# mratsim/constantine

Measured on NVIDIA H100. Metric: bls12_381_g1_msm_throughput, higher is better.
Workload: dtype u32

## Files before the change

### constantine_b200/_lib.py

```python
import ctypes
import os

_HERE = os.path.dirname(os.path.abspath(__file__))
LIB_PATH = os.environ.get("CTT_B200_LIB", os.path.join(_HERE, "lib", "libctt_b200_msm.so"))
_lib = None


class Stats(ctypes.Structure):
    _fields_ = [("c", ctypes.c_int), ("num_windows", ctypes.c_int),
                ("entries", ctypes.c_ulonglong), ("total_buckets", ctypes.c_ulonglong),
                ("kernel_launches", ctypes.c_int),
                ("ms_h2d", ctypes.c_float), ("ms_digits", ctypes.c_float), ("ms_sort", ctypes.c_float),
                ("ms_accumulate", ctypes.c_float), ("ms_fixup", ctypes.c_float), ("ms_reduce", ctypes.c_float),
                ("ms_d2h_tail", ctypes.c_float), ("ms_total", ctypes.c_float),
                ("groups", ctypes.c_int), ("slice_len", ctypes.c_int), ("affine_levels", ctypes.c_int),
                ("ms_affine", ctypes.c_float)]


def load():
    global _lib
    if _lib is not None:
        return _lib
    if not os.path.exists(LIB_PATH):
        raise RuntimeError(
# ... 27 lines not shown
    lib.ctt_b200_msm_batch_cached_bases.restype = ci
    lib.ctt_b200_bases_precompute_for.argtypes = [vp, sz, ci]
    lib.ctt_b200_bases_precompute_for.restype = ci
    lib.ctt_b200_sum_reduce_host.argtypes = [ci, ci, vp, vp, sz]
    lib.ctt_b200_sum_reduce_host.restype = ci
    lib.ctt_b200_last_stats.argtypes = [ctypes.POINTER(Stats)]
    lib.ctt_b200_last_stats.restype = None
    lib.ctt_b200_set_tuning.argtypes = [ci, ci, ci]
    lib.ctt_b200_set_tuning.restype = None
    lib.ctt_b200_set_concurrency.argtypes = [ci]
    lib.ctt_b200_set_concurrency.restype = None
    lib.ctt_b200_set_groups.argtypes = [ci]
    lib.ctt_b200_set_groups.restype = None
    lib.ctt_b200_set_affine_levels.argtypes = [ci]
    lib.ctt_b200_set_affine_levels.restype = None
    lib.ctt_b200_set_reduce_mode.argtypes = [ci]
    lib.ctt_b200_set_reduce_mode.restype = None
    lib.ctt_b200_set_input_chunks.argtypes = [ci]
    lib.ctt_b200_set_input_chunks.restype = None
    lib.ctt_b200_set_point_chunks.argtypes = [ci]
    lib.ctt_b200_set_point_chunks.restype = None
    lib.ctt_b200_set_stream.argtypes = [vp]
    lib.ctt_b200_set_stream.restype = None
    lib.ctt_b200_sm_count.argtypes = []
    lib.ctt_b200_sm_count.restype = ci
    lib.ctt_b200_set_devices.argtypes = [ctypes.POINTER(ci), ci]
    lib.ctt_b200_set_devices.restype = ci
    lib.ctt_b200_device_count.argtypes = []
    lib.ctt_b200_device_count.restype = ci
    lib.ctt_b200_test_field_op.argtypes = [ci, ci, vp, vp, vp, sz]
# ... 58 lines not shown
```

### constantine_b200/csrc/msm_affine.cuh

```cuda
#pragma once
#include "ec.cuh"
#include "field_inv.cuh"

namespace b200 {

constexpr int AFF_MAX_LEVELS = 8;
constexpr uint32_t AFF_NONE = 0xFFFFFFFFu;

static __global__ void k_bucket_bounds(const uint32_t* __restrict__ keys, size_t n, uint32_t no_key, uint32_t* head, uint32_t* tail) {
  size_t q = (size_t)blockIdx.x * blockDim.x + threadIdx.x;
  if (q >= n) return;
  const uint32_t key = keys[q];
  if (key >= no_key) return;
  if (q == 0 || keys[q - 1] != key) head[key] = (uint32_t)q;
  if (q + 1 == n || keys[q + 1] != key) tail[key] = (uint32_t)(q + 1);
}

constexpr int SCAN_THREADS = 256, SCAN_PER_THREAD = 4, SCAN_ITEMS = SCAN_THREADS * SCAN_PER_THREAD;

B200_DEV uint32_t block_exclusive_scan(uint32_t v, uint32_t& total, uint32_t* smem ) {
  const unsigned lane = threadIdx.x & 31u, warp = threadIdx.x >> 5;
  uint32_t inc = v;
#pragma unroll
  for (int d = 1; d < 32; d <<= 1) {
    uint32_t t = __shfl_up_sync(0xFFFFFFFFu, inc, d);
    if (lane >= (unsigned)d) inc += t;
  }
  __syncthreads();
  if (lane == 31u) smem[warp] = inc;
  __syncthreads();
  uint32_t base = 0, tot = 0;
#pragma unroll
  for (int w = 0; w < SCAN_THREADS / 32; w++) {
    const uint32_t s = smem[w];
    if ((unsigned)w < warp) base += s;
    tot += s;
  }
  total = tot;
  return base + inc - v;
}

B200_DEV uint32_t level_count(uint32_t n, int r) { return (n + (1u << r) - 1u) >> r; }

static __global__ void __launch_bounds__(SCAN_THREADS) k_level_blocksums(const uint32_t* __restrict__ head, const uint32_t* __restrict__ tail,
                                                                          uint32_t nb, int L, uint32_t nblk, uint32_t* blocksum ) {
  __shared__ uint32_t sm[SCAN_THREADS / 32 + 1];
  const uint32_t b0 = blockIdx.x * SCAN_ITEMS + threadIdx.x * SCAN_PER_THREAD;
  uint32_t cnt[SCAN_PER_THREAD];
#pragma unroll
  for (int k = 0; k < SCAN_PER_THREAD; k++) cnt[k] = (b0 + k < nb) ? tail[b0 + k] - head[b0 + k] : 0u;
  for (int r = 0; r <= L; r++) {
    uint32_t s = 0;
#pragma unroll
    for (int k = 0; k < SCAN_PER_THREAD; k++) s += level_count(cnt[k], r);
    uint32_t tot;
    block_exclusive_scan(s, tot, sm);
    if (threadIdx.x == 0) blocksum[(size_t)r * nblk + blockIdx.x] = tot;
  }
}

static __global__ void __launch_bounds__(SCAN_THREADS) k_level_scan(uint32_t* blocksum, uint32_t nblk, int L, uint32_t nb, uint32_t* off) {
  __shared__ uint32_t sm[SCAN_THREADS / 32 + 1];
  for (int r = 0; r <= L; r++) {
    uint32_t carry = 0;
    for (uint32_t base = 0; base < nblk; base += SCAN_THREADS) {
// ... 3 lines not shown
      const uint32_t ex = block_exclusive_scan(v, tot, sm);
      if (i < nblk) blocksum[(size_t)r * nblk + i] = carry + ex;
      carry += tot;
    }
    if (threadIdx.x == 0) off[(size_t)r * (nb + 1) + nb] = carry;
  }
}

static __global__ void __launch_bounds__(SCAN_THREADS) k_level_offsets(const uint32_t* __restrict__ head, const uint32_t* __restrict__ tail,
                                                                        uint32_t nb, int L, uint32_t nblk, const uint32_t* __restrict__ blocksum,
                                                                        uint32_t* off) {
  __shared__ uint32_t sm[SCAN_THREADS / 32 + 1];
  const uint32_t b0 = blockIdx.x * SCAN_ITEMS + threadIdx.x * SCAN_PER_THREAD;
  uint32_t cnt[SCAN_PER_THREAD];
#pragma unroll
  for (int k = 0; k < SCAN_PER_THREAD; k++) cnt[k] = (b0 + k < nb) ? tail[b0 + k] - head[b0 + k] : 0u;
  for (int r = 0; r <= L; r++) {
    uint32_t c[SCAN_PER_THREAD], s = 0;
#pragma unroll
    for (int k = 0; k < SCAN_PER_THREAD; k++) { c[k] = level_count(cnt[k], r); s += c[k]; }
    uint32_t tot;
    uint32_t ex = block_exclusive_scan(s, tot, sm) + blocksum[(size_t)r * nblk + blockIdx.x];
#pragma unroll
    for (int k = 0; k < SCAN_PER_THREAD; k++) {
      if (b0 + k < nb) off[(size_t)r * (nb + 1) + b0 + k] = ex;
      ex += c[k];
    }
  }
}

struct AffinePlan {
  uint2* plan0;
  uint32_t* plan[AFF_MAX_LEVELS];
  uint32_t* surv_keys;
  uint32_t* surv_vals;
};

static __global__ void k_affine_plan(const uint32_t* __restrict__ keys, const uint32_t* __restrict__ vals, size_t n, uint32_t no_key,
                                     const uint32_t* __restrict__ head, const uint32_t* __restrict__ tail,
                                     const uint32_t* __restrict__ off, uint32_t nb, int L, AffinePlan P) {
  size_t q = (size_t)blockIdx.x * blockDim.x + threadIdx.x;
  if (q >= n) return;
  const uint32_t b = keys[q];
  if (b >= no_key) return;
  const uint32_t h = head[b], i = (uint32_t)q - h, cnt = tail[b] - h;
  const size_t stride = (size_t)nb + 1;
  for (int r = 0; r < L; r++) {
    if (i & ((2u << r) - 1u)) break;
    const uint32_t p = off[(size_t)(r + 1) * stride + b] + (i >> (r + 1));
    const uint32_t s = i >> r;
    const bool has2 = s + 1u < level_count(cnt, r);
    if (r == 0) P.plan0[p] = make_uint2(vals[q], has2 ? vals[q + 1] : AFF_NONE);
    else P.plan[r][p] = (off[(size_t)r * stride + b] + s) | (has2 ? 0x80000000u : 0u);
  }
  if ((i & ((1u << L) - 1u)) == 0u) {
    const uint32_t ps = off[(size_t)L * stride + b] + (i >> L);
    P.surv_keys[ps] = b;
    P.surv_vals[ps] = ps;
  }
}

template <class T>
B200_DEV Aff<T> load_affine_rw(const uint32_t* base, size_t idx) {
  const uint32_t* p = base + idx * (2 * T::WORDS);
  Aff<T> a;
  load_words_rw(a.x, p);
  load_words_rw(a.y, p + T::WORDS);
  return a;
}
template <class T>
B200_DEV void store_affine(uint32_t* base, size_t idx, const Aff<T>& a) {
  uint32_t* p = base + idx * (2 * T::WORDS);
  store_words(p, a.x);
  store_words(p + T::WORDS, a.y);
// ... 291 lines not shown
```

### constantine_b200/csrc/msm_capi.cu

```cuda
#define CTT_B200_BUILDING_LIBRARY
#include "../../include/ctt_b200_msm.h"
#include "msm_hooks.cuh"
#include <thread>

namespace b200 {
B200_DECLARE_CURVE(Bls12381G1) B200_DECLARE_CURVE(Bn254G1) B200_DECLARE_CURVE(PallasEc) B200_DECLARE_CURVE(VestaEc)
B200_DECLARE_CURVE(Bls12381G2) B200_DECLARE_CURVE(Bn254G2)
B200_DECLARE_FIELD(Bls12381Fp) B200_DECLARE_FIELD(Bn254SnarksFp) B200_DECLARE_FIELD(PallasFp) B200_DECLARE_FIELD(VestaFp)
B200_DECLARE_FIELD(Bls12381Fr) B200_DECLARE_FIELD(Bn254SnarksFr) B200_DECLARE_FIELD(PallasFr) B200_DECLARE_FIELD(VestaFr)

struct Bases {
  int curve_id;
  size_t len;
  void* d_points;
  void* d_table = nullptr;
  int table_c = 0, table_W = 0;
};

void bases_view(const ctt_b200_bases* bases, const void** d_points, size_t* table_stride, int* force_c) {
  const Bases* b = reinterpret_cast<const Bases*>(bases);
  *d_points = b->d_table ? b->d_table : b->d_points;
  *table_stride = b->d_table ? b->len : 0;
  *force_c = b->d_table ? b->table_c : 0;
}
// ... 209 lines not shown
  if (slice_len < -1) cfg.tuning.slice_len = slice_len;
}

void ctt_b200_set_groups(int groups) {
  Config& cfg = config();
  std::lock_guard<std::mutex> lock(cfg.mu);
  cfg.tuning.groups = groups < 0 ? 0 : groups;
}

void ctt_b200_set_affine_levels(int levels) {
  Config& cfg = config();
  std::lock_guard<std::mutex> lock(cfg.mu);
  cfg.tuning.affine_levels = levels < 0 ? -1 : (levels > AFF_MAX_LEVELS ? AFF_MAX_LEVELS : levels);
}

void ctt_b200_set_reduce_mode(int mode) {
  Config& cfg = config();
  std::lock_guard<std::mutex> lock(cfg.mu);
  cfg.tuning.reduce_mode = mode == 1 ? 1 : 0;
}

void ctt_b200_set_input_chunks(int chunks) {
  Config& cfg = config();
  std::lock_guard<std::mutex> lock(cfg.mu);
  cfg.tuning.input_chunks = chunks < 0 ? 0 : chunks;
}

void ctt_b200_set_point_chunks(int pieces) {
  Config& cfg = config();
  std::lock_guard<std::mutex> lock(cfg.mu);
// ... 70 lines not shown
```

### constantine_b200/csrc/msm_engine.cuh

```cuda
#pragma once
#include <cstdio>
#include <cstdlib>
#include <cstring>
#include <atomic>
#include <condition_variable>
#include <functional>
#include <memory>
#include <mutex>
#include <thread>
#include <vector>
#include <cuda_runtime.h>
#include <cub/device/device_radix_sort.cuh>
#include <cub/device/device_scan.cuh>
#include "msm_kernels.cuh"
#include "msm_affine.cuh"
#include "host_field.hpp"

namespace b200 {

#define B200_CUDA_CHECK(expr)                                                                              \
  do {                                                                                                     \
    cudaError_t e__ = (expr);                                                                              \
    if (e__ != cudaSuccess) {                                                                              \
      fprintf(stderr, "[ctt_b200_msm] FATAL CUDA error %s (%s) at %s:%d -- no CPU fallback exists\n",      \
              cudaGetErrorName(e__), cudaGetErrorString(e__), __FILE__, __LINE__);                         \
      abort();                                                                                             \
    }                                                                                                      \
  } while (0)

template <class FpP, class FrP, int EXT>
// ... 19 lines not shown
using Bn254G1 = CurveDesc<Bn254SnarksFp, Bn254SnarksFr, 1>;
using PallasEc = CurveDesc<PallasFp, PallasFr, 1>;
using VestaEc = CurveDesc<VestaFp, VestaFr, 1>;
using Bls12381G2 = CurveDesc<Bls12381Fp, Bls12381Fr, 2>;
using Bn254G2 = CurveDesc<Bn254SnarksFp, Bn254SnarksFr, 2>;

struct Tuning {
  int force_c = 0;
  int reduce_chunk = 16;
  int slice_len = 0;
  int groups = 0;
  int affine_levels = -1;
  int reduce_mode = 0;
  int input_chunks = 0;
  int point_chunks = 0;
};

struct Stats {
  int c = 0, num_windows = 0;
  unsigned long long entries = 0;
  unsigned long long total_buckets = 0;
  int kernel_launches = 0;
  float ms_h2d = 0, ms_digits = 0, ms_sort = 0, ms_accumulate = 0, ms_fixup = 0, ms_reduce = 0, ms_d2h_tail = 0, ms_total = 0;
  int groups = 1, slice_len = 0;
  int affine_levels = 0;
  float ms_affine = 0;
};

inline int choose_window(size_t n, int bits, int coord_words = 12) {
  double best = 1e300;
// ... 59 lines not shown
  std::mutex mu;
  bool ready = false;
  int device = 0;
  int sm_count = 0;
  cudaStream_t stream = nullptr, copy_stream = nullptr;
  cudaStream_t user_stream = nullptr;
  cudaStream_t order_after = nullptr;
  cudaEvent_t ev_order = nullptr;
  cudaStream_t compute() const { return user_stream ? user_stream : stream; }
  cudaEvent_t ev[13];
  cudaEvent_t ev_points_ready;
  static constexpr int MAX_INPUT_CHUNKS = 8;
  cudaEvent_t ev_chunk[MAX_INPUT_CHUNKS];
  DeviceBuffer d_scalars, d_points, keys_a, keys_b, vals_a, vals_b, cub_tmp, buckets, part_pts[2], part_keys[2], red_a, red_b, red_planes, bounds;
  DeviceBuffer aff_head, aff_tail, aff_off, aff_blocksum, aff_plan[AFF_MAX_LEVELS], aff_work[2], aff_scratch, keys_s, vals_s, part_counts, part_starts, part_perm;
  DeviceBuffer kzg_poly, kzg_args;
  DeviceBuffer das_coefs, das_cells, das_u, das_proofs;
  void* h_result = nullptr;
  size_t h_result_cap = 0;
  static constexpr size_t STAGE_BYTES = 16u << 20;
  void* h_stage[2] = {nullptr, nullptr};
  cudaEvent_t ev_stage[2] = {nullptr, nullptr};
  void ensure_stage() {
    if (h_stage[0]) return;
    for (int i = 0; i < 2; i++) {
      B200_CUDA_CHECK(cudaMallocHost(&h_stage[i], STAGE_BYTES));
      B200_CUDA_CHECK(cudaEventCreateWithFlags(&ev_stage[i], cudaEventDisableTiming));
    }
  }
  void ensure_host(size_t bytes) {
// ... 28 lines not shown
  Tuning tuning;
  cudaStream_t user_stream = nullptr;
  int concurrency = 2;
  int primary_device = -1;
  std::vector<int> devices;
  bool devices_from_env_done = false;
  size_t multi_min_len = 1u << 15;
};
inline Config& config() {
  static Config* c = [] {
    Config* x = new Config;
    if (const char* v = getenv("CTT_B200_INPUT_CHUNKS")) x->tuning.input_chunks = atoi(v);
    if (const char* v = getenv("CTT_B200_POINT_CHUNKS")) x->tuning.point_chunks = atoi(v);
    if (const char* v = getenv("CTT_B200_REDUCE_MODE")) x->tuning.reduce_mode = atoi(v) == 1 ? 1 : 0;
    if (const char* v = getenv("CTT_B200_AFFINE_LEVELS")) x->tuning.affine_levels = atoi(v);
    if (const char* v = getenv("CTT_B200_FORCE_C")) x->tuning.force_c = atoi(v);
    return x;
  }();
  return *c;
}

struct DeviceGuard {
  int prev = -1;
  bool changed = false;
  explicit DeviceGuard(int dev) {
    B200_CUDA_CHECK(cudaGetDevice(&prev));
    if (dev >= 0 && prev != dev) { B200_CUDA_CHECK(cudaSetDevice(dev)); changed = true; }
  }
  DeviceGuard(const DeviceGuard&) = delete;
  DeviceGuard& operator=(const DeviceGuard&) = delete;
// ... 212 lines not shown
    int KACC = 64;
    uint32_t fit_threads;
    {
      static thread_local int acc_bps_cache[MAX_DEVICES] = {};
      int bps = acc_bps_cache[E.device];
      if (bps == 0) {
        B200_CUDA_CHECK(cudaOccupancyMaxActiveBlocksPerMultiprocessor(&bps, k_accumulate<T>, B200_ACC_THREADS, 0));
        if (bps < 1) bps = 1;
        acc_bps_cache[E.device] = bps;
      }
      fit_threads = (uint32_t)(E.sm_count * bps * B200_ACC_THREADS);
      if (E.tuning.slice_len > 0) { KACC = E.tuning.slice_len; fit_threads = 0; }
      else if (E.tuning.slice_len < 0) KACC = -E.tuning.slice_len;
    }
    st.slice_len = fit_threads ? accumulate_slice_len(acc_entries, fit_threads, KACC) : KACC;
    E.keys_a.ensure(entries * 4); E.keys_b.ensure(entries * 4);
    E.vals_a.ensure(entries * 4); E.vals_b.ensure(entries * 4);
    if (timed) B200_CUDA_CHECK(cudaEventRecord(E.ev[10], s));
    if (input_chunks && ch.ready) B200_CUDA_CHECK(cudaStreamWaitEvent(s, ch.ready, 0));
    {
      dim3 grid((unsigned)((ntot + 255) / 256)), block(256);
      const uint32_t msm_key_stride = (uint32_t)nws * B, psets = batch > 1 ? (uint32_t)point_sets : 1u;
      if (fr_mont)
        k_digits<typename C::FrParams, true><<<grid, block, 0, s>>>((const uint32_t*)sc, (uint32_t)ntot, plan, (uint32_t*)E.keys_a.ptr, (uint32_t*)E.vals_a.ptr,
                                                                     table_mode ? 0u : B, no_key, (uint32_t)table_stride, (uint32_t)nper, msm_key_stride, psets);
      else
        k_digits<typename C::FrParams, false><<<grid, block, 0, s>>>((const uint32_t*)sc, (uint32_t)ntot, plan, (uint32_t*)E.keys_a.ptr, (uint32_t*)E.vals_a.ptr,
                                                                      table_mode ? 0u : B, no_key, (uint32_t)table_stride, (uint32_t)nper, msm_key_stride, psets);
      launches++;
    }
    if (timed) B200_CUDA_CHECK(cudaEventRecord(E.ev[1], s));
    int end_bit = 1;
    while ((1ull << end_bit) <= (unsigned long long)no_key) end_bit++;
    cub::DoubleBuffer<uint32_t> dk((uint32_t*)E.keys_a.ptr, (uint32_t*)E.keys_b.ptr);
    cub::DoubleBuffer<uint32_t> dv((uint32_t*)E.vals_a.ptr, (uint32_t*)E.vals_b.ptr);
    {
      size_t tmp_bytes = 0;
      B200_CUDA_CHECK(cub::DeviceRadixSort::SortPairs(nullptr, tmp_bytes, dk, dv, (int64_t)entries, 0, end_bit, s));
      E.cub_tmp.ensure(tmp_bytes);
      B200_CUDA_CHECK(cub::DeviceRadixSort::SortPairs(E.cub_tmp.ptr, tmp_bytes, dk, dv, (int64_t)entries, 0, end_bit, s));
      launches += 2 + (end_bit + 7) / 8;
    }
    const uint32_t* keys = dk.Current();
    const uint32_t* vals = dv.Current();
    if (timed) B200_CUDA_CHECK(cudaEventRecord(E.ev[2], s));
    E.bounds.ensure((size_t)(nw + 1) * 8);
    k_window_bounds<<<(unsigned)((nw + 1 + 63) / 64), 64, 0, s>>>(keys, entries, B, nw, (unsigned long long*)E.bounds.ptr);
    launches++;
    size_t max_slices;
    {
      size_t set_cap = table_mode ? (size_t)nwd * nper : nper;
      if (AL) set_cap = (set_cap >> AL) + B + 1;
      const size_t list_cap = (size_t)nw * set_cap;
      max_slices = fit_threads ? accumulate_waves(list_cap, fit_threads, KACC) * fit_threads : (list_cap + KACC - 1) / KACC;
    }
    const size_t max_fix = (max_slices + KFIX - 1) / KFIX;
    E.part_pts[0].ensure(max_slices * XYZZ_BYTES); E.part_keys[0].ensure(max_slices * 4);
    E.part_pts[1].ensure(max_fix * XYZZ_BYTES); E.part_keys[1].ensure(max_fix * 4);
    const int PC = (point_chunks && !input_chunks) ? point_chunks->P : 0;
    auto piece_ready = [&](int q) {
      if (point_chunks->stage && *point_chunks->stage) (*point_chunks->stage)(q);
      B200_CUDA_CHECK(cudaStreamWaitEvent(s, point_chunks->ready[q], 0));
    };
    auto wait_for_points = [&]() {
      if (PC) { for (int q = 0; q < PC; q++) piece_ready(q); }
      else if (!input_chunks && ch.ready) B200_CUDA_CHECK(cudaStreamWaitEvent(s, ch.ready, 0));
    };
    const void* acc_points = pts;
    if (AL) {
      const uint32_t nb = (uint32_t)nbuckets;
      const uint32_t nblk = (nb + SCAN_ITEMS - 1) / SCAN_ITEMS;
      const size_t off_stride = (size_t)nb + 1;
      E.aff_head.ensure((size_t)nb * 4); E.aff_tail.ensure((size_t)nb * 4);
      E.aff_off.ensure((size_t)(AL + 1) * off_stride * 4);
      E.aff_blocksum.ensure((size_t)(AL + 1) * nblk * 4);
      E.aff_plan[0].ensure(level_cap(1) * 8);
      for (int r = 1; r < AL; r++) E.aff_plan[r].ensure(level_cap(r + 1) * 4);
      E.aff_work[1].ensure(level_cap(1) * AFF_BYTES);
      if (AL >= 2) E.aff_work[0].ensure(level_cap(2) * AFF_BYTES);
      E.keys_s.ensure(acc_entries * 4);
      E.vals_s.ensure(acc_entries * 4);
      static thread_local int bps_cache[MAX_DEVICES] = {};
      int bps = bps_cache[E.device];
      if (bps == 0) {
        B200_CUDA_CHECK(cudaOccupancyMaxActiveBlocksPerMultiprocessor(&bps, k_affine_pairs<T, true>, B200_AFF_THREADS, 0));
        int bps2 = 0;
        B200_CUDA_CHECK(cudaOccupancyMaxActiveBlocksPerMultiprocessor(&bps2, k_affine_pairs<T, false>, B200_AFF_THREADS, 0));
        if (bps2 < bps) bps = bps2;
        if (bps < 1) bps = 1;
        bps_cache[E.device] = bps;
      }
      const unsigned aff_grid = (unsigned)(E.sm_count * bps);
      const size_t aff_threads = (size_t)aff_grid * B200_AFF_THREADS;
      const size_t per_thread = (level_cap(1) + aff_threads - 1) / aff_threads;
      E.aff_scratch.ensure(per_thread * aff_threads * (size_t)T::WORDS * 4);
      uint32_t* head = (uint32_t*)E.aff_head.ptr;
      uint32_t* tail = (uint32_t*)E.aff_tail.ptr;
      uint32_t* off = (uint32_t*)E.aff_off.ptr;
      B200_CUDA_CHECK(cudaMemsetAsync(head, 0, (size_t)nb * 4, s));
      B200_CUDA_CHECK(cudaMemsetAsync(tail, 0, (size_t)nb * 4, s));
      B200_CUDA_CHECK(cudaMemsetAsync(E.keys_s.ptr, 0xFF, acc_entries * 4, s));
      const unsigned eb = (unsigned)((entries + 255) / 256);
      k_bucket_bounds<<<eb, 256, 0, s>>>(keys, entries, no_key, head, tail);
      k_level_blocksums<<<nblk, SCAN_THREADS, 0, s>>>(head, tail, nb, AL, nblk, (uint32_t*)E.aff_blocksum.ptr);
      k_level_scan<<<1, SCAN_THREADS, 0, s>>>((uint32_t*)E.aff_blocksum.ptr, nblk, AL, nb, off);
      k_level_offsets<<<nblk, SCAN_THREADS, 0, s>>>(head, tail, nb, AL, nblk, (const uint32_t*)E.aff_blocksum.ptr, off);
      AffinePlan aplan;
      aplan.plan0 = (uint2*)E.aff_plan[0].ptr;
      for (int r = 0; r < AFF_MAX_LEVELS; r++) aplan.plan[r] = (r >= 1 && r < AL) ? (uint32_t*)E.aff_plan[r].ptr : nullptr;
      aplan.surv_keys = (uint32_t*)E.keys_s.ptr;
      aplan.surv_vals = (uint32_t*)E.vals_s.ptr;
      k_affine_plan<<<eb, 256, 0, s>>>(keys, vals, entries, no_key, head, tail, off, nb, AL, aplan);
      const bool split0 = PC > 1;
      if (!split0) wait_for_points();
      for (int r = 0; r < AL; r++) {
        const uint32_t* total_ptr = off + (size_t)(r + 1) * off_stride + nb;
        uint32_t* dst = (uint32_t*)E.aff_work[(r + 1) & 1].ptr;
        if (r == 0 && split0) {
          const uint32_t Pq = (uint32_t)PC;
          const uint32_t nblk_p = (uint32_t)((level_cap(1) + PART_TILE - 1) / PART_TILE);
          E.part_counts.ensure((size_t)Pq * nblk_p * 4);
          E.part_starts.ensure((size_t)(Pq + 1) * 4);
          E.part_perm.ensure(level_cap(1) * 4);
          k_part_count<<<nblk_p, PART_THREADS, 0, s>>>((const uint2*)E.aff_plan[0].ptr, total_ptr, (uint32_t)nper, Pq, nblk_p, (uint32_t*)E.part_counts.ptr);
          k_part_scan<<<1, SCAN_THREADS, 0, s>>>((uint32_t*)E.part_counts.ptr, Pq, nblk_p, (uint32_t*)E.part_starts.ptr);
          k_part_scatter<<<nblk_p, PART_THREADS, 0, s>>>((const uint2*)E.aff_plan[0].ptr, total_ptr, (uint32_t)nper, Pq, nblk_p,
                                                          (const uint32_t*)E.part_counts.ptr, (uint32_t*)E.part_perm.ptr);
          for (int q = 0; q < PC; q++) {
            piece_ready(q);
            k_affine_pairs<T, true><<<aff_grid, B200_AFF_THREADS, 0, s>>>(E.aff_plan[0].ptr, total_ptr, (const uint32_t*)pts, dst, (uint4*)E.aff_scratch.ptr,
                                                                          (const uint32_t*)E.part_perm.ptr, (const uint32_t*)E.part_starts.ptr + q);
          }
          launches += 3 + PC - 1;
        } else if (r == 0)
          k_affine_pairs<T, true><<<aff_grid, B200_AFF_THREADS, 0, s>>>(E.aff_plan[0].ptr, total_ptr, (const uint32_t*)pts, dst, (uint4*)E.aff_scratch.ptr);
        else
          k_affine_pairs<T, false><<<aff_grid, B200_AFF_THREADS, 0, s>>>(E.aff_plan[r].ptr, total_ptr, (const uint32_t*)E.aff_work[r & 1].ptr, dst, (uint4*)E.aff_scratch.ptr);
      }
      keys = (const uint32_t*)E.keys_s.ptr;
      vals = (const uint32_t*)E.vals_s.ptr;
      acc_points = E.aff_work[AL & 1].ptr;
      k_window_bounds<<<(unsigned)((nw + 1 + 63) / 64), 64, 0, s>>>(keys, acc_entries, B, nw, (unsigned long long*)E.bounds.ptr);
      launches += 6 + AL;
      B200_CUDA_CHECK(cudaGetLastError());
      if (timed) B200_CUDA_CHECK(cudaEventRecord(E.ev[9], s));
    }
    st.affine_levels = AL;
    if (!AL) wait_for_points();
    {
      dim3 block(B200_ACC_THREADS), grid((unsigned)((max_slices + B200_ACC_THREADS - 1) / B200_ACC_THREADS));
      k_accumulate<T><<<grid, block, 0, s>>>(keys, vals, (const unsigned long long*)E.bounds.ptr, 0, nw, no_key, (const uint32_t*)acc_points,
                                             (uint32_t*)E.buckets.ptr, (uint32_t*)E.part_pts[0].ptr, (uint32_t*)E.part_keys[0].ptr, max_slices, KACC,
                                             into ? 1 : 0, fit_threads);
      launches++;
    }
    if (timed) B200_CUDA_CHECK(cudaEventRecord(E.ev[3], s));
    {
      size_t count = max_slices;
// ... 578 lines not shown
```

### constantine_b200/csrc/msm_kernels.cuh

```cuda
#pragma once
#include "ec.cuh"

namespace b200 {

struct DigitPlan {
  int bits;
  int c;
  int num_full;
  int num_windows;
  int excess;
  int top;
  uint32_t buckets_per_window;
  uint32_t total_buckets;
  int win_begin, win_end;
};

__device__ __forceinline__ uint32_t scalar_window(const uint32_t* k, int bit_index, int nbits) {
  int word = bit_index >> 5, pos = bit_index & 31;
  uint64_t lo = (word < 8) ? k[word] : 0u;
  uint64_t hi = (word + 1 < 8) ? k[word + 1] : 0u;
  uint64_t v = (lo | (hi << 32)) >> pos;
  return (uint32_t)v & ((1u << nbits) - 1u);
}

// ... 8 lines not shown
  if (w == p.num_full) {
    if (p.top == 0) signed_encode(scalar_window(k, 0, p.c) << 1, p.c, val, neg);
    else if (p.excess == 0) signed_encode(scalar_window(k, p.top - 1, p.c + 1), p.c, val, neg);
    else signed_encode(scalar_window(k, p.top - 1, p.excess + 1), p.excess + 1, val, neg);
  } else if (w == 0) {
    signed_encode(scalar_window(k, 0, p.c) << 1, p.c, val, neg);
  } else {
    signed_encode(scalar_window(k, w * p.c - 1, p.c + 1), p.c, val, neg);
  }
}

template <class FrParams, bool FR_MONT>
__global__ void __launch_bounds__(256) k_digits(const uint32_t* __restrict__ scalars, uint32_t n, DigitPlan plan,
                                                uint32_t* __restrict__ keys, uint32_t* __restrict__ vals,
                                                uint32_t key_stride, uint32_t no_key, uint32_t val_stride,
                                                uint32_t per, uint32_t msm_key_stride, uint32_t point_sets) {
  uint32_t i = blockIdx.x * blockDim.x + threadIdx.x;
  if (i >= n) return;
  uint32_t k[8];
  const uint4* src = reinterpret_cast<const uint4*>(scalars) + (size_t)i * 2;
  uint4 a = __ldg(src), b = __ldg(src + 1);
  k[0] = a.x; k[1] = a.y; k[2] = a.z; k[3] = a.w; k[4] = b.x; k[5] = b.y; k[6] = b.z; k[7] = b.w;
  if (FR_MONT) {
    static_assert(FrParams::N == 8, "256-bit scalar fields");
    uint32_t one[8] = {1, 0, 0, 0, 0, 0, 0, 0};
    fe_mul<FrParams>(k, k, one);
  }
  const uint32_t m = i / per;
  const uint32_t ref = (m % point_sets) * per + (i - m * per);
  const uint32_t key_base = m * msm_key_stride;
  for (int w = plan.win_begin; w < plan.win_end; w++) {
    uint32_t val, neg;
    window_digit(k, plan, w, val, neg);
    const uint32_t wl = (uint32_t)(w - plan.win_begin);
    size_t slot = (size_t)wl * n + i;
    keys[slot] = val ? key_base + wl * key_stride + (val - 1u) : no_key;
    vals[slot] = (wl * val_stride + ref) | (neg << 31);
  }
}

constexpr uint32_t KEY_NONE = 0xFFFFFFFFu;

#ifndef B200_ACC_MIN_BLOCKS
#define B200_ACC_MIN_BLOCKS 2
#endif
#ifndef B200_ACC_THREADS
#define B200_ACC_THREADS 128
#endif
#ifndef B200_ACC_MIN_SLICE
#define B200_ACC_MIN_SLICE 16
#endif
// ... 391 lines not shown
```

### include/ctt_b200_msm.h

```cpp
#ifndef CTT_B200_MSM_H
#define CTT_B200_MSM_H

#include <stddef.h>
#include <stdint.h>

#ifdef __cplusplus
extern "C" {
#endif

#ifndef __CTT_H_DATATYPES__
typedef size_t secret_word;
#endif

#ifndef __CTT_H_BIGINTS__
typedef struct { secret_word limbs[4]; } big255;
typedef struct { secret_word limbs[4]; } big254;
#endif
#ifndef __CTT_H_THREADPOOL__
typedef struct ctt_threadpool ctt_threadpool;
#endif
#ifndef __CTT_H_BLS12_381__
typedef struct { secret_word limbs[4]; } bls12_381_fr;
typedef struct { secret_word limbs[6]; } bls12_381_fp;
typedef struct { bls12_381_fp c[2]; } bls12_381_fp2;
// ... 141 lines not shown
  float ms_h2d, ms_digits, ms_sort, ms_accumulate, ms_fixup, ms_reduce, ms_d2h_tail, ms_total;
  int groups, slice_len;
  int affine_levels;
  float ms_affine;
} ctt_b200_stats;
void ctt_b200_last_stats(ctt_b200_stats* out);

void ctt_b200_set_tuning(int force_c, int reduce_chunk, int slice_len);

void ctt_b200_set_concurrency(int slots);

void ctt_b200_set_groups(int groups);

void ctt_b200_set_affine_levels(int levels);

void ctt_b200_set_reduce_mode(int mode);

void ctt_b200_set_input_chunks(int chunks);

void ctt_b200_set_point_chunks(int pieces);

void ctt_b200_set_stream(void* cuda_stream);

int ctt_b200_sm_count(void);

int ctt_b200_set_devices(const int* device_ids, int count);
int ctt_b200_device_count(void);

#ifndef __CTT_H_DATATYPES__
typedef uint8_t byte;
// ... 51 lines not shown
```

Before: 104.7.

## Shrink radix sort key range and add sort-free bucket planning front path

For single-MSM affine runs, digit keys are repacked as (digit << wbits) | window, and the radix sort covers only the digit bits. This relies on the sort being stable to keep window order inside each digit, and it cuts the number of sort passes. Bucket bounds and plan kernels now map packed keys back to bucket indices. The plan kernel handles four entries per thread with vector loads, and window bounds are skipped when affine levels are on. An optional path, off by default, replaces the global sort with per-tile shared-memory histograms and a block radix sort that scatter straight into the affine plan.

```diff
diff --git a/constantine_b200/_lib.py b/constantine_b200/_lib.py
--- a/constantine_b200/_lib.py
+++ b/constantine_b200/_lib.py
@@ -65,6 +65,8 @@
     lib.ctt_b200_set_groups.restype = None
     lib.ctt_b200_set_affine_levels.argtypes = [ci]
     lib.ctt_b200_set_affine_levels.restype = None
+    lib.ctt_b200_set_affine_front.argtypes = [ci]
+    lib.ctt_b200_set_affine_front.restype = None
     lib.ctt_b200_set_reduce_mode.argtypes = [ci]
     lib.ctt_b200_set_reduce_mode.restype = None
     lib.ctt_b200_set_input_chunks.argtypes = [ci]
diff --git a/constantine_b200/csrc/msm_affine.cuh b/constantine_b200/csrc/msm_affine.cuh
--- a/constantine_b200/csrc/msm_affine.cuh
+++ b/constantine_b200/csrc/msm_affine.cuh
@@ -7,13 +7,19 @@
 constexpr int AFF_MAX_LEVELS = 8;
 constexpr uint32_t AFF_NONE = 0xFFFFFFFFu;
 
-static __global__ void k_bucket_bounds(const uint32_t* __restrict__ keys, size_t n, uint32_t no_key, uint32_t* head, uint32_t* tail) {
+B200_DEV uint32_t bucket_of_key(uint32_t key, uint32_t wbits, uint32_t B) {
+  return wbits ? (key & ((1u << wbits) - 1u)) * B + (key >> wbits) : key;
+}
+
+static __global__ void k_bucket_bounds(const uint32_t* __restrict__ keys, size_t n, uint32_t no_key, uint32_t wbits, uint32_t B,
+                                       uint32_t* head, uint32_t* tail) {
   size_t q = (size_t)blockIdx.x * blockDim.x + threadIdx.x;
   if (q >= n) return;
   const uint32_t key = keys[q];
   if (key >= no_key) return;
-  if (q == 0 || keys[q - 1] != key) head[key] = (uint32_t)q;
-  if (q + 1 == n || keys[q + 1] != key) tail[key] = (uint32_t)(q + 1);
+  const uint32_t b = bucket_of_key(key, wbits, B);
+  if (q == 0 || keys[q - 1] != key) head[b] = (uint32_t)q;
+  if (q + 1 == n || keys[q + 1] != key) tail[b] = (uint32_t)(q + 1);
 }
 
 constexpr int SCAN_THREADS = 256, SCAN_PER_THREAD = 4, SCAN_ITEMS = SCAN_THREADS * SCAN_PER_THREAD;
@@ -41,6 +47,10 @@
 }
 
 B200_DEV uint32_t level_count(uint32_t n, int r) { return (n + (1u << r) - 1u) >> r; }
+
+B200_DEV uint32_t run_length(const uint32_t* __restrict__ head, const uint32_t* __restrict__ tail, uint32_t b) {
+  return head ? tail[b] - head[b] : tail[b];
+}
 
 static __global__ void __launch_bounds__(SCAN_THREADS) k_level_blocksums(const uint32_t* __restrict__ head, const uint32_t* __restrict__ tail,
                                                                           uint32_t nb, int L, uint32_t nblk, uint32_t* blocksum ) {
@@ -48,7 +58,7 @@
   const uint32_t b0 = blockIdx.x * SCAN_ITEMS + threadIdx.x * SCAN_PER_THREAD;
   uint32_t cnt[SCAN_PER_THREAD];
 #pragma unroll
-  for (int k = 0; k < SCAN_PER_THREAD; k++) cnt[k] = (b0 + k < nb) ? tail[b0 + k] - head[b0 + k] : 0u;
+  for (int k = 0; k < SCAN_PER_THREAD; k++) cnt[k] = (b0 + k < nb) ? run_length(head, tail, b0 + k) : 0u;
   for (int r = 0; r <= L; r++) {
     uint32_t s = 0;
 #pragma unroll
@@ -82,7 +92,7 @@
   const uint32_t b0 = blockIdx.x * SCAN_ITEMS + threadIdx.x * SCAN_PER_THREAD;
   uint32_t cnt[SCAN_PER_THREAD];
 #pragma unroll
-  for (int k = 0; k < SCAN_PER_THREAD; k++) cnt[k] = (b0 + k < nb) ? tail[b0 + k] - head[b0 + k] : 0u;
+  for (int k = 0; k < SCAN_PER_THREAD; k++) cnt[k] = (b0 + k < nb) ? run_length(head, tail, b0 + k) : 0u;
   for (int r = 0; r <= L; r++) {
     uint32_t c[SCAN_PER_THREAD], s = 0;
 #pragma unroll
@@ -104,21 +114,20 @@
   uint32_t* surv_vals;
 };
 
-static __global__ void k_affine_plan(const uint32_t* __restrict__ keys, const uint32_t* __restrict__ vals, size_t n, uint32_t no_key,
-                                     const uint32_t* __restrict__ head, const uint32_t* __restrict__ tail,
-                                     const uint32_t* __restrict__ off, uint32_t nb, int L, AffinePlan P) {
-  size_t q = (size_t)blockIdx.x * blockDim.x + threadIdx.x;
-  if (q >= n) return;
-  const uint32_t b = keys[q];
-  if (b >= no_key) return;
+B200_DEV void plan_entry(size_t q, uint32_t key, uint32_t v, uint32_t v_next, uint32_t no_key, uint32_t wbits, uint32_t B,
+                         const uint32_t* __restrict__ head, const uint32_t* __restrict__ tail, const uint32_t* __restrict__ off,
+                         uint32_t nb, int L, const AffinePlan& P) {
+  if (key >= no_key) return;
+  const uint32_t b = bucket_of_key(key, wbits, B);
   const uint32_t h = head[b], i = (uint32_t)q - h, cnt = tail[b] - h;
   const size_t stride = (size_t)nb + 1;
-  for (int r = 0; r < L; r++) {
-    if (i & ((2u << r) - 1u)) break;
+#pragma unroll
+  for (int r = 0; r < AFF_MAX_LEVELS; r++) {
+    if (r >= L || (i & ((2u << r) - 1u))) break;
     const uint32_t p = off[(size_t)(r + 1) * stride + b] + (i >> (r + 1));
     const uint32_t s = i >> r;
     const bool has2 = s + 1u < level_count(cnt, r);
-    if (r == 0) P.plan0[p] = make_uint2(vals[q], has2 ? vals[q + 1] : AFF_NONE);
+    if (r == 0) P.plan0[p] = make_uint2(v, has2 ? v_next : AFF_NONE);
     else P.plan[r][p] = (off[(size_t)r * stride + b] + s) | (has2 ? 0x80000000u : 0u);
   }
   if ((i & ((1u << L) - 1u)) == 0u) {
@@ -126,6 +135,30 @@
     P.surv_keys[ps] = b;
     P.surv_vals[ps] = ps;
   }
+}
+
+constexpr int PLAN_ITEMS = 4;
+static_assert(PLAN_ITEMS == 4, "k_affine_plan unpacks one uint4 of keys and of refs");
+static __global__ void k_affine_plan(const uint32_t* __restrict__ keys, const uint32_t* __restrict__ vals, size_t n, uint32_t no_key,
+                                     uint32_t wbits, uint32_t B, const uint32_t* __restrict__ head, const uint32_t* __restrict__ tail,
+                                     const uint32_t* __restrict__ off, uint32_t nb, int L, AffinePlan P) {
+  const size_t q0 = ((size_t)blockIdx.x * blockDim.x + threadIdx.x) * PLAN_ITEMS;
+  if (q0 >= n) return;
+  uint32_t k[PLAN_ITEMS], v[PLAN_ITEMS + 1];
+  if (q0 + PLAN_ITEMS <= n) {
+    const uint4 k4 = *reinterpret_cast<const uint4*>(keys + q0), v4 = *reinterpret_cast<const uint4*>(vals + q0);
+    k[0] = k4.x; k[1] = k4.y; k[2] = k4.z; k[3] = k4.w;
+    v[0] = v4.x; v[1] = v4.y; v[2] = v4.z; v[3] = v4.w;
+  } else {
+#pragma unroll
+    for (int j = 0; j < PLAN_ITEMS; j++) {
+      k[j] = q0 + j < n ? keys[q0 + j] : no_key;
+      v[j] = q0 + j < n ? vals[q0 + j] : 0u;
+    }
+  }
+  v[PLAN_ITEMS] = (q0 + PLAN_ITEMS < n && k[PLAN_ITEMS - 1] < no_key) ? vals[q0 + PLAN_ITEMS] : 0u;
+#pragma unroll
+  for (int j = 0; j < PLAN_ITEMS; j++) plan_entry(q0 + j, k[j], v[j], v[j + 1], no_key, wbits, B, head, tail, off, nb, L, P);
 }
 
 template <class T>
diff --git a/constantine_b200/csrc/msm_capi.cu b/constantine_b200/csrc/msm_capi.cu
--- a/constantine_b200/csrc/msm_capi.cu
+++ b/constantine_b200/csrc/msm_capi.cu
@@ -247,6 +247,12 @@
   cfg.tuning.affine_levels = levels < 0 ? -1 : (levels > AFF_MAX_LEVELS ? AFF_MAX_LEVELS : levels);
 }
 
+void ctt_b200_set_affine_front(int mode) {
+  Config& cfg = config();
+  std::lock_guard<std::mutex> lock(cfg.mu);
+  cfg.tuning.affine_front = mode < 0 ? -1 : 0;
+}
+
 void ctt_b200_set_reduce_mode(int mode) {
   Config& cfg = config();
   std::lock_guard<std::mutex> lock(cfg.mu);
diff --git a/constantine_b200/csrc/msm_engine.cuh b/constantine_b200/csrc/msm_engine.cuh
--- a/constantine_b200/csrc/msm_engine.cuh
+++ b/constantine_b200/csrc/msm_engine.cuh
@@ -14,6 +14,7 @@
 #include <cub/device/device_scan.cuh>
 #include "msm_kernels.cuh"
 #include "msm_affine.cuh"
+#include "msm_front.cuh"
 #include "host_field.hpp"
 
 namespace b200 {
@@ -63,6 +64,7 @@
   int reduce_mode = 0;
   int input_chunks = 0;
   int point_chunks = 0;
+  int affine_front = 0;
 };
 
 struct Stats {
@@ -152,6 +154,7 @@
   cudaEvent_t ev_chunk[MAX_INPUT_CHUNKS];
   DeviceBuffer d_scalars, d_points, keys_a, keys_b, vals_a, vals_b, cub_tmp, buckets, part_pts[2], part_keys[2], red_a, red_b, red_planes, bounds;
   DeviceBuffer aff_head, aff_tail, aff_off, aff_blocksum, aff_plan[AFF_MAX_LEVELS], aff_work[2], aff_scratch, keys_s, vals_s, part_counts, part_starts, part_perm;
+  DeviceBuffer front_counts, front_scalars;
   DeviceBuffer kzg_poly, kzg_args;
   DeviceBuffer das_coefs, das_cells, das_u, das_proofs;
   void* h_result = nullptr;
@@ -210,6 +213,7 @@
     if (const char* v = getenv("CTT_B200_POINT_CHUNKS")) x->tuning.point_chunks = atoi(v);
     if (const char* v = getenv("CTT_B200_REDUCE_MODE")) x->tuning.reduce_mode = atoi(v) == 1 ? 1 : 0;
     if (const char* v = getenv("CTT_B200_AFFINE_LEVELS")) x->tuning.affine_levels = atoi(v);
+    if (const char* v = getenv("CTT_B200_AFFINE_FRONT")) x->tuning.affine_front = atoi(v) < 0 ? -1 : 0;
     if (const char* v = getenv("CTT_B200_FORCE_C")) x->tuning.force_c = atoi(v);
     return x;
   }();
@@ -452,39 +456,50 @@
       else if (E.tuning.slice_len < 0) KACC = -E.tuning.slice_len;
     }
     st.slice_len = fit_threads ? accumulate_slice_len(acc_entries, fit_threads, KACC) : KACC;
-    E.keys_a.ensure(entries * 4); E.keys_b.ensure(entries * 4);
-    E.vals_a.ensure(entries * 4); E.vals_b.ensure(entries * 4);
+    const bool front = AL > 0 && batch == 1 && !table_mode && E.tuning.affine_front != 0 && c <= FRONT_MAX_C;
+    if (!front) {
+      E.keys_a.ensure(entries * 4); E.keys_b.ensure(entries * 4);
+      E.vals_a.ensure(entries * 4); E.vals_b.ensure(entries * 4);
+    }
     if (timed) B200_CUDA_CHECK(cudaEventRecord(E.ev[10], s));
     if (input_chunks && ch.ready) B200_CUDA_CHECK(cudaStreamWaitEvent(s, ch.ready, 0));
-    {
+    const uint32_t* keys = nullptr;
+    const uint32_t* vals = nullptr;
+    uint32_t wbits = 0;
+    if (AL > 0 && batch == 1 && !table_mode) while ((1 << wbits) < nwd) wbits++;
+    const uint32_t sort_no_key = wbits ? (B << wbits) : no_key;
+    if (!front) {
       dim3 grid((unsigned)((ntot + 255) / 256)), block(256);
       const uint32_t msm_key_stride = (uint32_t)nws * B, psets = batch > 1 ? (uint32_t)point_sets : 1u;
       if (fr_mont)
         k_digits<typename C::FrParams, true><<<grid, block, 0, s>>>((const uint32_t*)sc, (uint32_t)ntot, plan, (uint32_t*)E.keys_a.ptr, (uint32_t*)E.vals_a.ptr,
-                                                                     table_mode ? 0u : B, no_key, (uint32_t)table_stride, (uint32_t)nper, msm_key_stride, psets);
+                                                                     table_mode ? 0u : B, sort_no_key, (uint32_t)table_stride, (uint32_t)nper, msm_key_stride, psets, wbits);
       else
         k_digits<typename C::FrParams, false><<<grid, block, 0, s>>>((const uint32_t*)sc, (uint32_t)ntot, plan, (uint32_t*)E.keys_a.ptr, (uint32_t*)E.vals_a.ptr,
-                                                                      table_mode ? 0u : B, no_key, (uint32_t)table_stride, (uint32_t)nper, msm_key_stride, psets);
+                                                                      table_mode ? 0u : B, sort_no_key, (uint32_t)table_stride, (uint32_t)nper, msm_key_stride, psets, wbits);
       launches++;
-    }
-    if (timed) B200_CUDA_CHECK(cudaEventRecord(E.ev[1], s));
-    int end_bit = 1;
-    while ((1ull << end_bit) <= (unsigned long long)no_key) end_bit++;
-    cub::DoubleBuffer<uint32_t> dk((uint32_t*)E.keys_a.ptr, (uint32_t*)E.keys_b.ptr);
-    cub::DoubleBuffer<uint32_t> dv((uint32_t*)E.vals_a.ptr, (uint32_t*)E.vals_b.ptr);
-    {
-      size_t tmp_bytes = 0;
-      B200_CUDA_CHECK(cub::DeviceRadixSort::SortPairs(nullptr, tmp_bytes, dk, dv, (int64_t)entries, 0, end_bit, s));
-      E.cub_tmp.ensure(tmp_bytes);
-      B200_CUDA_CHECK(cub::DeviceRadixSort::SortPairs(E.cub_tmp.ptr, tmp_bytes, dk, dv, (int64_t)entries, 0, end_bit, s));
-      launches += 2 + (end_bit + 7) / 8;
-    }
-    const uint32_t* keys = dk.Current();
-    const uint32_t* vals = dv.Current();
-    if (timed) B200_CUDA_CHECK(cudaEventRecord(E.ev[2], s));
+      if (timed) B200_CUDA_CHECK(cudaEventRecord(E.ev[1], s));
+      int end_bit = 1;
+      while ((1ull << end_bit) <= (unsigned long long)sort_no_key) end_bit++;
+      const int begin_bit = (int)wbits;
+      cub::DoubleBuffer<uint32_t> dk((uint32_t*)E.keys_a.ptr, (uint32_t*)E.keys_b.ptr);
+      cub::DoubleBuffer<uint32_t> dv((uint32_t*)E.vals_a.ptr, (uint32_t*)E.vals_b.ptr);
+      {
+        size_t tmp_bytes = 0;
+        B200_CUDA_CHECK(cub::DeviceRadixSort::SortPairs(nullptr, tmp_bytes, dk, dv, (int64_t)entries, begin_bit, end_bit, s));
+        E.cub_tmp.ensure(tmp_bytes);
+        B200_CUDA_CHECK(cub::DeviceRadixSort::SortPairs(E.cub_tmp.ptr, tmp_bytes, dk, dv, (int64_t)entries, begin_bit, end_bit, s));
+        launches += 2 + (end_bit - begin_bit + 7) / 8;
+      }
+      keys = dk.Current();
+      vals = dv.Current();
+      if (timed) B200_CUDA_CHECK(cudaEventRecord(E.ev[2], s));
+    }
     E.bounds.ensure((size_t)(nw + 1) * 8);
-    k_window_bounds<<<(unsigned)((nw + 1 + 63) / 64), 64, 0, s>>>(keys, entries, B, nw, (unsigned long long*)E.bounds.ptr);
-    launches++;
+    if (!AL) {
+      k_window_bounds<<<(unsigned)((nw + 1 + 63) / 64), 64, 0, s>>>(keys, entries, B, nw, (unsigned long long*)E.bounds.ptr);
+      launches++;
+    }
     size_t max_slices;
     {
       size_t set_cap = table_mode ? (size_t)nwd * nper : nper;
@@ -509,7 +524,8 @@
       const uint32_t nb = (uint32_t)nbuckets;
       const uint32_t nblk = (nb + SCAN_ITEMS - 1) / SCAN_ITEMS;
       const size_t off_stride = (size_t)nb + 1;
-      E.aff_head.ensure((size_t)nb * 4); E.aff_tail.ensure((size_t)nb * 4);
+      if (!front) E.aff_head.ensure((size_t)nb * 4);
+      E.aff_tail.ensure((size_t)nb * 4);
       E.aff_off.ensure((size_t)(AL + 1) * off_stride * 4);
       E.aff_blocksum.ensure((size_t)(AL + 1) * nblk * 4);
       E.aff_plan[0].ensure(level_cap(1) * 8);
@@ -535,20 +551,53 @@
       uint32_t* head = (uint32_t*)E.aff_head.ptr;
       uint32_t* tail = (uint32_t*)E.aff_tail.ptr;
       uint32_t* off = (uint32_t*)E.aff_off.ptr;
-      B200_CUDA_CHECK(cudaMemsetAsync(head, 0, (size_t)nb * 4, s));
-      B200_CUDA_CHECK(cudaMemsetAsync(tail, 0, (size_t)nb * 4, s));
-      B200_CUDA_CHECK(cudaMemsetAsync(E.keys_s.ptr, 0xFF, acc_entries * 4, s));
-      const unsigned eb = (unsigned)((entries + 255) / 256);
-      k_bucket_bounds<<<eb, 256, 0, s>>>(keys, entries, no_key, head, tail);
-      k_level_blocksums<<<nblk, SCAN_THREADS, 0, s>>>(head, tail, nb, AL, nblk, (uint32_t*)E.aff_blocksum.ptr);
-      k_level_scan<<<1, SCAN_THREADS, 0, s>>>((uint32_t*)E.aff_blocksum.ptr, nblk, AL, nb, off);
-      k_level_offsets<<<nblk, SCAN_THREADS, 0, s>>>(head, tail, nb, AL, nblk, (const uint32_t*)E.aff_blocksum.ptr, off);
       AffinePlan aplan;
       aplan.plan0 = (uint2*)E.aff_plan[0].ptr;
       for (int r = 0; r < AFF_MAX_LEVELS; r++) aplan.plan[r] = (r >= 1 && r < AL) ? (uint32_t*)E.aff_plan[r].ptr : nullptr;
       aplan.surv_keys = (uint32_t*)E.keys_s.ptr;
       aplan.surv_vals = (uint32_t*)E.vals_s.ptr;
-      k_affine_plan<<<eb, 256, 0, s>>>(keys, vals, entries, no_key, head, tail, off, nb, AL, aplan);
+      B200_CUDA_CHECK(cudaMemsetAsync(E.keys_s.ptr, 0xFF, acc_entries * 4, s));
+      if (front) {
+        const uint32_t ntiles = (uint32_t)((nper + FRONT_TILE - 1) / FRONT_TILE);
+        const unsigned fblocks = ntiles * (unsigned)nwd;
+        const size_t hist_bytes = (size_t)B * 4;
+        E.front_counts.ensure((size_t)nwd * ntiles * B * 4);
+        static thread_local bool smem_set[MAX_DEVICES] = {};
+        if (!smem_set[E.device]) {
+          const int max_hist = (1 << (FRONT_MAX_C - 1)) * 4;
+          B200_CUDA_CHECK(cudaFuncSetAttribute(k_front_count, cudaFuncAttributeMaxDynamicSharedMemorySize, max_hist));
+          B200_CUDA_CHECK(cudaFuncSetAttribute(k_front_scatter, cudaFuncAttributeMaxDynamicSharedMemorySize, max_hist));
+          smem_set[E.device] = true;
+        }
+        const uint32_t* fsc = (const uint32_t*)sc;
+        if (fr_mont) {
+          E.front_scalars.ensure(nper * 32);
+          k_scalars_canonical<typename C::FrParams><<<(unsigned)((nper + 255) / 256), 256, 0, s>>>(fsc, (uint32_t)nper, (uint32_t*)E.front_scalars.ptr);
+          fsc = (const uint32_t*)E.front_scalars.ptr;
+          launches++;
+        }
+        uint32_t* counts = (uint32_t*)E.front_counts.ptr;
+        k_front_count<<<fblocks, FRONT_THREADS, hist_bytes, s>>>(fsc, (uint32_t)nper, plan, ntiles, counts);
+        if (timed) B200_CUDA_CHECK(cudaEventRecord(E.ev[1], s));
+        k_front_tile_scan<<<(nb + 255) / 256, 256, 0, s>>>(counts, nb, B, ntiles, tail);
+        k_level_blocksums<<<nblk, SCAN_THREADS, 0, s>>>(nullptr, tail, nb, AL, nblk, (uint32_t*)E.aff_blocksum.ptr);
+        k_level_scan<<<1, SCAN_THREADS, 0, s>>>((uint32_t*)E.aff_blocksum.ptr, nblk, AL, nb, off);
+        k_level_offsets<<<nblk, SCAN_THREADS, 0, s>>>(nullptr, tail, nb, AL, nblk, (const uint32_t*)E.aff_blocksum.ptr, off);
+        k_front_scatter<<<fblocks, FRONT_THREADS, hist_bytes, s>>>(fsc, (uint32_t)nper, plan, ntiles, counts, off, nb, aplan.plan0);
+        k_front_levels<<<(unsigned)(((nb + 31) / 32 * 32 + 255) / 256), 256, 0, s>>>(off, nb, AL, aplan);
+        launches += 7;
+        if (timed) B200_CUDA_CHECK(cudaEventRecord(E.ev[2], s));
+      } else {
+        B200_CUDA_CHECK(cudaMemsetAsync(head, 0, (size_t)nb * 4, s));
+        B200_CUDA_CHECK(cudaMemsetAsync(tail, 0, (size_t)nb * 4, s));
+        const unsigned eb = (unsigned)((entries + 255) / 256);
+        k_bucket_bounds<<<eb, 256, 0, s>>>(keys, entries, sort_no_key, wbits, B, head, tail);
+        k_level_blocksums<<<nblk, SCAN_THREADS, 0, s>>>(head, tail, nb, AL, nblk, (uint32_t*)E.aff_blocksum.ptr);
+        k_level_scan<<<1, SCAN_THREADS, 0, s>>>((uint32_t*)E.aff_blocksum.ptr, nblk, AL, nb, off);
+        k_level_offsets<<<nblk, SCAN_THREADS, 0, s>>>(head, tail, nb, AL, nblk, (const uint32_t*)E.aff_blocksum.ptr, off);
+        k_affine_plan<<<(unsigned)((entries + 256 * PLAN_ITEMS - 1) / (256 * PLAN_ITEMS)), 256, 0, s>>>(keys, vals, entries, sort_no_key, wbits, B, head, tail, off, nb, AL, aplan);
+        launches += 5;
+      }
       const bool split0 = PC > 1;
       if (!split0) wait_for_points();
       for (int r = 0; r < AL; r++) {
@@ -579,7 +628,7 @@
       vals = (const uint32_t*)E.vals_s.ptr;
       acc_points = E.aff_work[AL & 1].ptr;
       k_window_bounds<<<(unsigned)((nw + 1 + 63) / 64), 64, 0, s>>>(keys, acc_entries, B, nw, (unsigned long long*)E.bounds.ptr);
-      launches += 6 + AL;
+      launches += 1 + AL;
       B200_CUDA_CHECK(cudaGetLastError());
       if (timed) B200_CUDA_CHECK(cudaEventRecord(E.ev[9], s));
     }
diff --git a/constantine_b200/csrc/msm_front.cuh b/constantine_b200/csrc/msm_front.cuh
--- /dev/null
+++ b/constantine_b200/csrc/msm_front.cuh
@@ -0,0 +1,156 @@
+#pragma once
+#include <cub/block/block_radix_sort.cuh>
+#include "msm_kernels.cuh"
+#include "msm_affine.cuh"
+
+namespace b200 {
+
+constexpr int FRONT_THREADS = 512, FRONT_IPT = 8, FRONT_CHUNK = FRONT_THREADS * FRONT_IPT;
+constexpr uint32_t FRONT_TILE = 1u << 16;
+constexpr int FRONT_MAX_C = 16;
+constexpr uint32_t FRONT_NO_BUCKET = 0xFFFFFFFFu;
+
+template <class FrParams>
+__global__ void __launch_bounds__(256) k_scalars_canonical(const uint32_t* __restrict__ in, uint32_t n, uint32_t* __restrict__ out) {
+  const uint32_t i = blockIdx.x * blockDim.x + threadIdx.x;
+  if (i >= n) return;
+  static_assert(FrParams::N == 8, "256-bit scalar fields");
+  uint32_t k[8];
+  const uint4* src = reinterpret_cast<const uint4*>(in) + (size_t)i * 2;
+  const uint4 a = __ldg(src), b = __ldg(src + 1);
+  k[0] = a.x; k[1] = a.y; k[2] = a.z; k[3] = a.w; k[4] = b.x; k[5] = b.y; k[6] = b.z; k[7] = b.w;
+  const uint32_t one[8] = {1, 0, 0, 0, 0, 0, 0, 0};
+  fe_mul<FrParams>(k, k, one);
+  uint4* dst = reinterpret_cast<uint4*>(out) + (size_t)i * 2;
+  dst[0] = make_uint4(k[0], k[1], k[2], k[3]);
+  dst[1] = make_uint4(k[4], k[5], k[6], k[7]);
+}
+
+B200_DEV uint32_t front_bucket(const uint32_t* __restrict__ scalars, uint32_t i, const DigitPlan& plan, int w, uint32_t& ref_sign) {
+  uint32_t val, neg;
+  window_digit(scalars + (size_t)i * 8, plan, w, val, neg);
+  ref_sign = i | (neg << 31);
+  return val ? val - 1u : FRONT_NO_BUCKET;
+}
+
+static __global__ void __launch_bounds__(FRONT_THREADS) k_front_count(const uint32_t* __restrict__ scalars, uint32_t n, DigitPlan plan,
+                                                                      uint32_t ntiles, uint32_t* __restrict__ counts) {
+  extern __shared__ uint32_t hist[];
+  const uint32_t B = plan.buckets_per_window;
+  const uint32_t ntl = ntiles, wl = blockIdx.x / ntl, tile = blockIdx.x % ntl;
+  for (uint32_t b = threadIdx.x; b < B; b += FRONT_THREADS) hist[b] = 0;
+  __syncthreads();
+  const uint32_t i0 = tile * FRONT_TILE, i1 = min(n, i0 + FRONT_TILE);
+  for (uint32_t i = i0 + threadIdx.x; i < i1; i += FRONT_THREADS) {
+    uint32_t rs;
+    const uint32_t b = front_bucket(scalars, i, plan, plan.win_begin + (int)wl, rs);
+    if (b != FRONT_NO_BUCKET) atomicAdd(&hist[b], 1u);
+  }
+  __syncthreads();
+  uint32_t* out = counts + ((size_t)wl * ntiles + tile) * B;
+  for (uint32_t b = threadIdx.x; b < B; b += FRONT_THREADS) out[b] = hist[b];
+}
+
+static __global__ void k_front_tile_scan(uint32_t* counts, uint32_t nb, uint32_t B, uint32_t ntiles, uint32_t* __restrict__ run) {
+  const uint32_t g = blockIdx.x * blockDim.x + threadIdx.x;
+  if (g >= nb) return;
+  uint32_t* p = counts + (size_t)(g / B) * ntiles * B + (g % B);
+  uint32_t sum = 0;
+  for (uint32_t t = 0; t < ntiles; t++) {
+    const uint32_t c = p[(size_t)t * B];
+    p[(size_t)t * B] = sum;
+    sum += c;
+  }
+  run[g] = sum;
+}
+
+static __global__ void __launch_bounds__(FRONT_THREADS, 1) k_front_scatter(const uint32_t* __restrict__ scalars, uint32_t n, DigitPlan plan,
+                                                                        uint32_t ntiles, const uint32_t* __restrict__ tile_base,
+                                                                        const uint32_t* __restrict__ off, uint32_t nb, uint2* plan0) {
+  using Sort = cub::BlockRadixSort<uint32_t, FRONT_THREADS, FRONT_IPT, uint32_t>;
+  __shared__ typename Sort::TempStorage sort_tmp;
+  __shared__ uint32_t first_key[FRONT_THREADS], last_key[FRONT_THREADS];
+  extern __shared__ uint32_t cursor[];
+  const uint32_t B = plan.buckets_per_window;
+  const uint32_t ntl = ntiles, wl = blockIdx.x / ntl, tile = blockIdx.x % ntl;
+  const uint32_t* base = tile_base + ((size_t)wl * ntiles + tile) * B;
+  for (uint32_t b = threadIdx.x; b < B; b += FRONT_THREADS) cursor[b] = base[b];
+  const uint32_t* off0 = off;
+  const uint32_t* off1 = off + (size_t)nb + 1;
+  const uint32_t gbase = wl * B;
+  const int w = plan.win_begin + (int)wl;
+  const int sort_bits = plan.c;
+  uint32_t* words = reinterpret_cast<uint32_t*>(plan0);
+  const uint32_t i0 = tile * FRONT_TILE, i1 = min(n, i0 + FRONT_TILE);
+  for (uint32_t c0 = i0; c0 < i1; c0 += FRONT_CHUNK) {
+    uint32_t key[FRONT_IPT], val[FRONT_IPT];
+#pragma unroll
+    for (int k = 0; k < FRONT_IPT; k++) {
+      const uint32_t i = c0 + threadIdx.x * FRONT_IPT + k;
+      key[k] = B;
+      val[k] = 0;
+      if (i < i1) {
+        const uint32_t b = front_bucket(scalars, i, plan, w, val[k]);
+        if (b != FRONT_NO_BUCKET) key[k] = b;
+      }
+    }
+    __syncthreads();
+    Sort(sort_tmp).Sort(key, val, 0, sort_bits);
+    first_key[threadIdx.x] = key[0];
+    last_key[threadIdx.x] = key[FRONT_IPT - 1];
+    __syncthreads();
+    const uint32_t prev_last = threadIdx.x ? last_key[threadIdx.x - 1] : B;
+    const uint32_t next_first = threadIdx.x + 1 < FRONT_THREADS ? first_key[threadIdx.x + 1] : B;
+#pragma unroll
+    for (int k = 0; k < FRONT_IPT; k++) {
+      const uint32_t prev = k ? key[k - 1] : prev_last;
+      if (key[k] < B && key[k] != prev) cursor[key[k]] -= threadIdx.x * FRONT_IPT + k;
+    }
+    __syncthreads();
+    uint32_t rank[FRONT_IPT];
+#pragma unroll
+    for (int k = 0; k < FRONT_IPT; k++) rank[k] = key[k] < B ? cursor[key[k]] + threadIdx.x * FRONT_IPT + k : 0u;
+    __syncthreads();
+#pragma unroll
+    for (int k = 0; k < FRONT_IPT; k++) {
+      const uint32_t next = k + 1 < FRONT_IPT ? key[k + 1] : next_first;
+      if (key[k] < B && key[k] != next) cursor[key[k]] = rank[k] + 1u;
+    }
+#pragma unroll
+    for (int k = 0; k < FRONT_IPT; k++) {
+      if (key[k] >= B) continue;
+      const uint32_t g = gbase + key[k], r = rank[k];
+      const size_t p = (size_t)off1[g] + (r >> 1);
+      if (r & 1u) {
+        words[2 * p + 1] = val[k];
+      } else {
+        words[2 * p] = val[k];
+        if (r + 1u == off0[g + 1] - off0[g]) words[2 * p + 1] = AFF_NONE;
+      }
+    }
+  }
+}
+
+static __global__ void k_front_levels(const uint32_t* __restrict__ off, uint32_t nb, int L, AffinePlan P) {
+  const uint32_t lane = threadIdx.x & 31u;
+  const uint32_t g0 = (uint32_t)(((size_t)blockIdx.x * blockDim.x + threadIdx.x) >> 5) * 32u;
+  if (g0 >= nb) return;
+  const uint32_t g1 = min(nb, g0 + 32u);
+  const size_t stride = (size_t)nb + 1;
+  for (uint32_t g = g0; g < g1; g++) {
+#pragma unroll
+    for (int r = 1; r < AFF_MAX_LEVELS; r++) {
+      if (r >= L) break;
+      const uint32_t src = off[(size_t)r * stride + g], n_r = off[(size_t)r * stride + g + 1] - src;
+      const uint32_t dst = off[(size_t)(r + 1) * stride + g], n_next = off[(size_t)(r + 1) * stride + g + 1] - dst;
+      for (uint32_t j = lane; j < n_next; j += 32u) P.plan[r][dst + j] = (src + 2u * j) | (2u * j + 1u < n_r ? 0x80000000u : 0u);
+    }
+    const uint32_t s0 = off[(size_t)L * stride + g], ns = off[(size_t)L * stride + g + 1] - s0;
+    for (uint32_t j = lane; j < ns; j += 32u) {
+      P.surv_keys[s0 + j] = g;
+      P.surv_vals[s0 + j] = s0 + j;
+    }
+  }
+}
+
+}
diff --git a/constantine_b200/csrc/msm_kernels.cuh b/constantine_b200/csrc/msm_kernels.cuh
--- a/constantine_b200/csrc/msm_kernels.cuh
+++ b/constantine_b200/csrc/msm_kernels.cuh
@@ -46,7 +46,7 @@
 __global__ void __launch_bounds__(256) k_digits(const uint32_t* __restrict__ scalars, uint32_t n, DigitPlan plan,
                                                 uint32_t* __restrict__ keys, uint32_t* __restrict__ vals,
                                                 uint32_t key_stride, uint32_t no_key, uint32_t val_stride,
-                                                uint32_t per, uint32_t msm_key_stride, uint32_t point_sets) {
+                                                uint32_t per, uint32_t msm_key_stride, uint32_t point_sets, uint32_t wbits = 0) {
   uint32_t i = blockIdx.x * blockDim.x + threadIdx.x;
   if (i >= n) return;
   uint32_t k[8];
@@ -66,7 +66,8 @@
     window_digit(k, plan, w, val, neg);
     const uint32_t wl = (uint32_t)(w - plan.win_begin);
     size_t slot = (size_t)wl * n + i;
-    keys[slot] = val ? key_base + wl * key_stride + (val - 1u) : no_key;
+    if (wbits) keys[slot] = val ? ((val - 1u) << wbits) | wl : no_key;
+    else keys[slot] = val ? key_base + wl * key_stride + (val - 1u) : no_key;
     vals[slot] = (wl * val_stride + ref) | (neg << 31);
   }
 }
diff --git a/include/ctt_b200_msm.h b/include/ctt_b200_msm.h
--- a/include/ctt_b200_msm.h
+++ b/include/ctt_b200_msm.h
@@ -179,6 +179,8 @@
 
 void ctt_b200_set_affine_levels(int levels);
 
+void ctt_b200_set_affine_front(int mode);
+
 void ctt_b200_set_reduce_mode(int mode);
 
 void ctt_b200_set_input_chunks(int chunks);
```

Result: faster. 109.0, median of 6 (+4.1%).
